# LiuShenLan/global_body_planner

Measured on AMD Instinct MI355X. Metric: valid extend-attempts/sec + time-to-first-solution, 1024×1024 rough_terrain, higher is better.
Workload: dtype f64; 1 GPU; config 3: synth-rough-1024, 262,144-attempt batch per GPU, isValidStateActionPair[Reverse] 50/50; terrain=synth-rough-1024, batch_per_gpu=262144, global_batch=262144, seed=20251018, kernel=persistent, waves=2, adaptive=False, terrain_storage=f32, parallelism=shard1 (no collective on the data path)

## Files before the change

### global_body_planner_amd/_lib.py

```python
import ctypes
import os

_HERE = os.path.dirname(os.path.abspath(__file__))
LIB_PATH = os.path.join(_HERE, "lib", "libgbp.so")

OK = 0
FLIGHT, STANCE, CONNECT_STANCE = 0, 1, 2
FORWARD, REVERSE = 0, 1
TRAPPED, ADVANCED, REACHED = 0, 1, 2
NUM_GEN_STATES = 6
F_VALID, F_OOD, F_NAN, F_SNEW_SET, F_TNEW_SET, F_FRAGILE, F_LIMIT, F_RESOLVED = 1, 2, 4, 8, 16, 32, 64, 128
MAX_SAMPLES = 7000
F_STAGE_SHIFT = 8
F_STAGE_MASK = 0xF << F_STAGE_SHIFT
STORAGE_AUTO, STORAGE_F32, STORAGE_F64 = 0, 1, 2
OPT_KERNEL, OPT_BLOCK, OPT_WAVES, OPT_LDS_COORDS, OPT_HELPERS = 1, 2, 4, 5, 8
OPT_AFFINE_COORDS, OPT_COORD_MODE, OPT_XCD_MAP, OPT_FAST_RCP, OPT_FRAGILE_EPS = 9, 10, 13, 14, 15
OPT_NN_STATS = 18
PLAN_HALT_TARGETS, PLAN_HALT_EXTEND, PLAN_HALT_CONNECT = 1, 2, 4
PLAN_HALT_STAR, PLAN_HALT_STAR_PAIRS = 8, 16
KERNEL_DIRECT, KERNEL_PERSISTENT = 0, 1

EXPORTS = [
    "gbp_version", "gbp_status_string", "gbp_device_count", "gbp_device_alloc",
    "gbp_device_free", "gbp_memcpy_h2d", "gbp_memcpy_d2h", "gbp_stream_synchronize",
    "gbp_terrain_create", "gbp_terrain_destroy", "gbp_terrain_info",
    "gbp_terrain_set_option", "gbp_terrain_get_option",
    "gbp_height_batch_dev", "gbp_height_batch_host",
    "gbp_normal_batch_dev", "gbp_normal_batch_host",
    "gbp_valid_states_dev", "gbp_valid_states_host",
    "gbp_validate_pairs_dev", "gbp_validate_pairs_host",
    "gbp_sample_states_dev", "gbp_sample_states_host", "gbp_sample_actions_dev",
    "gbp_sample_actions_host", "gbp_terrain_set_sampling", "gbp_terrain_get_sampling",
    "gbp_sample_states_dir_dev", "gbp_sample_states_dir_host", "gbp_sample_actions_dir_dev",
    "gbp_sample_actions_dir_host",
    "gbp_extend_batch_dev", "gbp_extend_batch_host",
    "gbp_nearest_batch_dev", "gbp_nearest_batch_host",
    "gbp_neighbors_batch_dev", "gbp_neighbors_batch_host", "gbp_knn_batch_dev", "gbp_knn_batch_host",
    "gbp_knn_yaw_batch_dev", "gbp_knn_yaw_batch_host", "gbp_host_yaw",
    "gbp_resolve_fragile_host", "gbp_resolve_fragile_states_host", "gbp_extend_resolve_host",
    "gbp_stream_create", "gbp_stream_destroy",
    "gbp_tree_create", "gbp_tree_destroy", "gbp_tree_init", "gbp_tree_reserve", "gbp_tree_capacity",
    "gbp_tree_size", "gbp_tree_read", "gbp_tree_append_host", "gbp_tree_load_host",
    "gbp_tree_device_ptrs", "gbp_vertex_map_order", "gbp_vertex_map_rank",
    "gbp_plan_ws_create", "gbp_plan_ws_destroy", "gbp_plan_reset", "gbp_plan_half_dev",
    "gbp_plan_halves_dev", "gbp_plan_star_config", "gbp_plan_stage_timing", "gbp_plan_stage_times",
    "gbp_plan_status_read", "gbp_plan_resolve_host", "gbp_extend_tree_dev",
    "gbp_extend_tree_finish_dev", "gbp_extend_tree_host", "gbp_tree_nearest_dev",
]


class Sampling(ctypes.Structure):
    _fields_ = [("state_flag", ctypes.c_int32), ("state_speed_direction", ctypes.c_int32),
                ("state_p", ctypes.c_double), ("action_flag", ctypes.c_int32),
                ("reserved", ctypes.c_int32), ("action_p", ctypes.c_double)]


def sampling(state_flag=False, state_p=0.05, speed_direction=False, action_flag=False,
             action_p=0.15):
    return Sampling(int(bool(state_flag)), int(bool(speed_direction)), float(state_p),
                    int(bool(action_flag)), 0, float(action_p))


class GbpError(RuntimeError):
    def __init__(self, status, what=""):
        self.status = status
        msg = _lib.gbp_status_string(status).decode() if _lib is not None else str(status)
        super().__init__(f"{what}: gbp status {status} ({msg})")


_lib = None


def load(path=None):
    global _lib
    if path is None and _lib is not None:
        return _lib
    p = path or LIB_PATH
    if not os.path.exists(p):
        raise FileNotFoundError(
            f"{p} is missing: build the HIP engine first "
            "(python -c 'import __graft_entry__ as g; g.build()')")
    L = ctypes.CDLL(p)
    P, I, I64, U64, SZ = ctypes.c_void_p, ctypes.c_int, ctypes.c_int64, ctypes.c_uint64, ctypes.c_size_t
    sig = {
        "gbp_version": (I, []),
        "gbp_status_string": (ctypes.c_char_p, [I]),
        "gbp_device_count": (I, [P]),
        "gbp_device_alloc": (I, [I, SZ, P]),
        "gbp_device_free": (I, [P]),
        "gbp_memcpy_h2d": (I, [P, P, SZ, P]),
        "gbp_memcpy_d2h": (I, [P, P, SZ, P]),
        "gbp_stream_synchronize": (I, [P]),
        "gbp_terrain_create": (I, [I, I, I, P, P, P, P, P, P, I, P]),
        "gbp_terrain_destroy": (I, [P]),
        "gbp_terrain_info": (I, [P, P, P, P, P, P]),
        "gbp_terrain_set_option": (I, [P, I, I64]),
        "gbp_terrain_get_option": (I, [P, I, P]),
        "gbp_height_batch_dev": (I, [P, I64, P, P, P, P, P]),
        "gbp_height_batch_host": (I, [P, I64, P, P, P, P]),
        "gbp_normal_batch_dev": (I, [P, I64, P, P, P, P]),
        "gbp_normal_batch_host": (I, [P, I64, P, P, P]),
        "gbp_valid_states_dev": (I, [P, I64, P, P, I, P, P, P, P]),
        "gbp_valid_states_host": (I, [P, I64, P, P, I, P, P, P]),
        "gbp_validate_pairs_dev": (I, [P, I64, P, P, P, I, I, P, P, P, P, P, P]),
        "gbp_validate_pairs_host": (I, [P, I64, P, P, P, I, I, P, P, P, P, P]),
        "gbp_sample_states_dev": (I, [P, I64, U64, U64, I64, I, I, P, P, P]),
        "gbp_sample_actions_dev": (I, [I64, P, U64, U64, I64, P, P]),
        "gbp_sample_states_host": (I, [P, I64, U64, U64, I64, I, I, P, P]),
        "gbp_sample_actions_host": (I, [P, I64, P, U64, U64, I64, P]),
        "gbp_terrain_set_sampling": (I, [P, P]),
        "gbp_terrain_get_sampling": (I, [P, P]),
        "gbp_sample_states_dir_dev": (I, [P, I64, U64, U64, I64, P, P, P, P, P]),
        "gbp_sample_states_dir_host": (I, [P, I64, U64, U64, I64, P, P, P, P]),
        "gbp_sample_actions_dir_dev": (I, [P, I64, P, P, P, P, I, P, U64, U64, I64, P, P]),
        "gbp_sample_actions_dir_host": (I, [P, I64, P, P, P, P, I, P, U64, U64, I64, P]),
        "gbp_extend_batch_dev": (I, [P, I64, P, P, P, I, I, U64, I64, P, P, P, P, P, P, P]),
        "gbp_extend_batch_host": (I, [P, I64, P, P, P, I, I, U64, I64, P, P, P, P, P, P]),
        "gbp_resolve_fragile_host": (I, [P, I64, P, P, P, I, I, P, P, P, P, P, P]),
        "gbp_resolve_fragile_states_host": (I, [P, I64, P, P, I, P, P, P, P]),
        "gbp_extend_resolve_host": (I, [P, I64, P, P, P, I, I, U64, I64, P, P, P, P, P, P, P]),
        "gbp_stream_create": (I, [I, P]),
        "gbp_stream_destroy": (I, [P]),
        "gbp_tree_create": (I, [I, I64, P]),
        "gbp_tree_destroy": (I, [P]),
        "gbp_tree_init": (I, [P, P, P]),
        "gbp_tree_reserve": (I, [P, I64, P]),
        "gbp_tree_capacity": (I, [P, P]),
        "gbp_tree_size": (I, [P, P, P]),
        "gbp_tree_read": (I, [P, I64, I64, P, P, P, P, P]),
        "gbp_tree_append_host": (I, [P, I64, P, P, P, P]),
        "gbp_tree_load_host": (I, [P, I64, P, P, P, P]),
        "gbp_vertex_map_order": (I, [I64, P]),
        "gbp_vertex_map_rank": (I, [I64, I64, P]),
        "gbp_tree_device_ptrs": (I, [P, P, P]),
        "gbp_plan_ws_create": (I, [P, I64, P]),
        "gbp_plan_ws_destroy": (I, [P]),
        "gbp_plan_reset": (I, [P, I64, P]),
        "gbp_plan_half_dev": (I, [P, P, P, P, ctypes.c_int32, I, I64, U64, U64, I64, I, I, P]),
        "gbp_plan_halves_dev": (I, [P, P, P, P, ctypes.c_int32, ctypes.c_int32, I64, U64, U64, U64,
                                    I, I, P]),
        "gbp_plan_status_read": (I, [P, P, P]),
        "gbp_plan_star_config": (I, [P, I, ctypes.c_double, I64, I64]),
        "gbp_plan_stage_timing": (I, [P, I]),
        "gbp_plan_stage_times": (I, [P, P, I, P, I]),
        "gbp_plan_resolve_host": (I, [P, P, P, P, I, I64, I, P, P, P]),
        "gbp_extend_tree_dev": (I, [P, P, P, I64, P, P, I, I, U64, I64, P, P, P]),
        "gbp_extend_tree_finish_dev": (I, [P, P, P, I64, I, P, P, P]),
        "gbp_extend_tree_host": (I, [P, P, P, I64, P, I, I, U64, I64, P, P, P]),
        "gbp_tree_nearest_dev": (I, [P, P, I64, P, P, P]),
        "gbp_nearest_batch_dev": (I, [I64, P, I64, P, P, P, P]),
# ... 28 lines not shown
```

### global_body_planner_amd/csrc/gbp_engine.hip

```cpp
#pragma clang fp contract(off)

#include <hip/hip_runtime.h>
#include <stdint.h>
#include <string.h>

#include <cstring>

#include <algorithm>
#include <cmath>
#include <mutex>
#include <new>
#include <vector>

#include "gbp.h"
#include "gbp_device.h"
#include "gbp_lane.h"
#include "gbp_um_order.h"
#include "gbp_internal.h"
#include "host/gbp_host_check.h"

using namespace gbp;

namespace {

// ... 62 lines not shown
    for (int k = 0; k < 8; k++) s[k] = states[8 * i + k];
    Acc acc{0, 0, 0};
    const bool v = is_valid_state(T, s, phase ? phase[i] : phase_all, acc);
    if (valid) valid[i] = v;
    if (flags) flags[i] = acc.flags | (v ? GBP_F_VALID : 0u);
    if (counts) counts[i] = (acc.G & 0xFFFFu) | (acc.V << 16);
  }
}

extern __shared__ double gbp_smem[];

template <class ZT, bool ADAPTIVE, int W, int CM>
__global__ __launch_bounds__(256, W) void k_validate_direct(
    TerrainView<ZT> T0, int64_t n, const double *__restrict__ S, const double *__restrict__ A,
    const uint8_t *__restrict__ dir, int dir_all, uint8_t *__restrict__ valid,
    double *__restrict__ s_new, double *__restrict__ t_new, uint32_t *__restrict__ flags,
    uint32_t *__restrict__ counts) {
  const TerrainView<ZT> T = CM == 1 ? stage_coords(T0, gbp_smem) : T0;
  const int64_t i = blockIdx.x * (int64_t)blockDim.x + threadIdx.x;
  if (i >= n) return;
  double s[8], a[10], sn[8];
#pragma unroll
  for (int k = 0; k < 8; k++) s[k] = S[8 * i + k];
#pragma unroll
  for (int k = 0; k < 10; k++) a[k] = A[10 * i + k];
  double tn = 0;
  Acc acc{0, 0, 0};
  uint32_t f = 0;
  const int d = dir ? dir[i] : dir_all;
  const bool v = (d == GBP_FORWARD) ? pair_forward<ZT, ADAPTIVE>(T, s, a, sn, tn, acc, f)
                                    : pair_reverse<ZT, ADAPTIVE>(T, s, a, sn, tn, acc, f);
  f |= acc.flags | (v ? GBP_F_VALID : 0u);
  if (valid) valid[i] = v;
  if (s_new && (f & GBP_F_SNEW_SET)) {
#pragma unroll
    for (int k = 0; k < 8; k++) s_new[8 * i + k] = sn[k];
  }
  if (t_new && (f & GBP_F_TNEW_SET)) t_new[i] = tn;
  flags[i] = f;
  if (counts) counts[i] = (acc.G & 0xFFFFu) | (acc.V << 16);
}



struct SnewRec {
  int idx, kind;
  double p;
};
constexpr int SN_RING = 2 * 64;

struct XBox {
  int seq, ack, fin, n_idle;
  unsigned long long act;
  int st[64];
  uint32_t vb[64], r0[64], r1[64];
  double t[64], ts[64];
};

#ifdef GBP_LOOP_PROF
__device__ unsigned long long gbp_loop_prof[8192 * 12];
#define LP_T(v) const unsigned long long v = __builtin_readcyclecounter()
#define LP_ADD(k, a, b) lp[k] += (b) - (a)
#else
#define LP_T(v)
#define LP_ADD(k, a, b)
#endif

template <class ZT, bool ADAPTIVE, int W, int CM, bool ONE>
__global__ __launch_bounds__(512, W) void k_validate_persistent(
    TerrainView<ZT> T0, int n, const double *__restrict__ S, const double *__restrict__ A,
    const uint8_t *__restrict__ dir, int dir_all, uint8_t *__restrict__ valid,
    double *__restrict__ s_new, double *__restrict__ t_new, uint32_t *__restrict__ flags,
    uint32_t *__restrict__ counts, const int *__restrict__ n_dev, int helpers, int xcd_map) {
#ifndef GBP_LDS_TERRAIN
  const TerrainView<ZT> T = CM == 1 ? stage_coords(T0, gbp_smem) : T0;
#else
  TerrainView<ZT> T = CM == 1 ? stage_coords(T0, gbp_smem) : T0;
  {
    ZT *zl = (ZT *)((SnewRec *)(gbp_smem + (CM == 1 ? (T0.nx + T0.ny + 1) & ~1 : 0) +
                                (size_t)blockDim.x * SA_ROW) +
                    (blockDim.x / WAVE) * SN_RING);
    const int nz = 2 * (T0.nx - 1) * T0.ny;
    typedef ZT zpair __attribute__((ext_vector_type(2)));
    for (int i = threadIdx.x; i < nz / 2; i += blockDim.x)
      ((zpair *)zl)[i] = ((const zpair *)T0.z)[i];
    __syncthreads();
#ifndef GBP_LDS_TERRAIN_STAGE_ONLY
    T.z = zl;
#endif
  }
#endif
  if (n_dev) n = *n_dev;
  const int lane = threadIdx.x & (WAVE - 1);
  const unsigned long long lt_mask = (1ull << lane) - 1ull;
  double *const SA = gbp_smem + (CM == 1 ? (T0.nx + T0.ny + 1) & ~1 : 0);
  double *const wave_rows = SA + (size_t)(threadIdx.x & ~(WAVE - 1)) * SA_ROW;
  SnewRec *const ring = (SnewRec *)(SA + (size_t)blockDim.x * SA_ROW) + (threadIdx.x / WAVE) * SN_RING;
  int ring_n = 0;
  auto flush = [&](int cnt) {
    if (lane < cnt) {
      const SnewRec r = ring[lane];
      double sv[8], av[10], o[8];
#pragma unroll
      for (int k = 0; k < 8; k++) sv[k] = S[8 * (size_t)r.idx + k];
#pragma unroll
      for (int k = 0; k < 10; k++) av[k] = A[10 * (size_t)r.idx + k];
      sample_state(sv, av,
                   r.kind == SN_STANCE_S ? ST_FWD_STANCE
                                         : (r.kind == SN_FLIGHT_B ? ST_FWD_LAND : ST_REV_STANCE),
                   r.p, o);
#pragma unroll
      for (int k = 0; k < 8; k++) s_new[8 * (size_t)r.idx + k] = o[k];
    }
  };
#ifdef GBP_XWAVE
  XBox *const xbox = (XBox *)((SnewRec *)(SA + (size_t)blockDim.x * SA_ROW) + (blockDim.x / WAVE) * SN_RING);
  const int wv = threadIdx.x / WAVE;
  XBox *const mybox = xbox + wv;
  XBox *const pbox = xbox + (wv ^ 1);
  const bool has_partner = (wv ^ 1) < (int)(blockDim.x / WAVE);
  double *const partner_rows = SA + (size_t)((wv ^ 1) * WAVE) * SA_ROW;
  if (lane == 0) {
    mybox->seq = 0;
    mybox->ack = 0;
    mybox->fin = 0;
  }
  __syncthreads();
  int myseq = 0, served = 0;
  bool fin_sent = false;
#endif
  Lane L;
  L.s = SA + (size_t)threadIdx.x * SA_ROW;
  L.a = L.s + 8;
  L.stage = ST_IDLE;
  unsigned int cur, end;
  {
    const unsigned int waves = gridDim.x * (blockDim.x / WAVE);
    const unsigned int wg = (xcd_map && (gridDim.x & 7u) == 0)
                                ? (blockIdx.x & 7u) * (gridDim.x >> 3) + (blockIdx.x >> 3)
                                : blockIdx.x;
    const unsigned int wid = wg * (blockDim.x / WAVE) + threadIdx.x / WAVE;
    cur = (unsigned int)(((unsigned long long)n * wid) / waves);
    end = (unsigned int)(((unsigned long long)n * (wid + 1)) / waves);
  }
#ifdef GBP_LOOP_PROF
  unsigned long long lp[12] = {0, 0, 0, 0, 0, 0, 0, 0, 0, 0, 0, 0};
  lp[8] = __builtin_amdgcn_s_memrealtime();
  LP_T(lp_start);
#endif
  for (;;) {
    LP_T(t0);
    const bool need = L.stage == ST_IDLE;
    unsigned long long m = __ballot(need);
    if (m && cur < end) {
      const unsigned int take = min(end - cur, (unsigned int)__popcll(m));
      const unsigned int rank = (unsigned int)__popcll(m & lt_mask);
      const bool mine = need && rank < take;
      if (mine) {
        const unsigned int i = cur + rank;
        L.idx = (int)i;
#pragma unroll
        for (int k = 0; k < 8; k++) L.s[k] = S[8 * (size_t)i + k];
#pragma unroll
        for (int k = 0; k < 10; k++) L.a[k] = A[10 * (size_t)i + k];
        L.f = 0;
        L.acc = Acc{0, 0, 0};
        L.snew_kind = SN_NONE;
        L.tnew_set = 0;
        const int d = dir ? dir[i] : dir_all;
        enter_stage(L, d == GBP_FORWARD ? ST_FWD_STANCE : ST_REV_FLIGHT);
      }
      cur += take;
    }
    const unsigned long long act = __ballot(L.stage != ST_IDLE);
#ifdef GBP_XWAVE
    bool serve = false;
    if (!act) {
      if (!has_partner) break;
      if (!fin_sent) {
        __builtin_amdgcn_fence(__ATOMIC_RELEASE, "workgroup");
        if (lane == 0) __hip_atomic_store(&mybox->fin, 1, __ATOMIC_RELEASE, __HIP_MEMORY_SCOPE_WORKGROUP);
        fin_sent = true;
      }
      int pseq, pfin;
      for (;;) {
        pseq = __builtin_amdgcn_readfirstlane(
            __hip_atomic_load(&pbox->seq, __ATOMIC_ACQUIRE, __HIP_MEMORY_SCOPE_WORKGROUP));
        pfin = __builtin_amdgcn_readfirstlane(
            __hip_atomic_load(&pbox->fin, __ATOMIC_ACQUIRE, __HIP_MEMORY_SCOPE_WORKGROUP));
        if (pseq != served || pfin) break;
        __builtin_amdgcn_s_sleep(1);
      }
      if (pseq == served) break;
      __builtin_amdgcn_fence(__ATOMIC_ACQUIRE, "workgroup");
      served = pseq;
      serve = true;
    }
#else
    if (!act) break;
#endif
    LP_T(t1);
    LP_ADD(0, t0, t1);
    const bool owner = L.stage != ST_IDLE;
    asm volatile("" ::: "memory");
    const int n_act = __popcll(act);
    const bool tail = helpers && n_act < WAVE;
    int st = L.stage, slot = 0;
    const double *ps = L.s;
    double t_eval = owner ? stage_time(L) : 0.0;
    uint32_t vbase = L.acc.V;
    bool has = owner;
#ifdef GBP_XWAVE
    bool xhelp = false;
    if (tail && !serve && has_partner) {
      xhelp = __builtin_amdgcn_readfirstlane(
                  __hip_atomic_load(&pbox->fin, __ATOMIC_ACQUIRE, __HIP_MEMORY_SCOPE_WORKGROUP)) != 0;
      if (xhelp) {
        mybox->st[lane] = L.stage;
        mybox->t[lane] = L.t;
        mybox->ts[lane] = L.ts;
        mybox->vb[lane] = L.acc.V;
        if (lane == 0) {
          mybox->act = act;
          mybox->n_idle = WAVE - n_act;
        }
        __builtin_amdgcn_fence(__ATOMIC_RELEASE, "workgroup");
        myseq++;
        if (lane == 0) __hip_atomic_store(&mybox->seq, myseq, __ATOMIC_RELEASE, __HIP_MEMORY_SCOPE_WORKGROUP);
      }
    }
    if (serve) {
      const unsigned long long pact = pbox->act;
      const int pn = __popcll(pact);
      const int j = pbox->n_idle + lane;
      const int src = nth_set_bit(pact, j % pn);
      slot = 1 + j / pn;
      ps = partner_rows + src * SA_ROW;
      st = pbox->st[src];
      double t = pbox->t[src], ts = pbox->ts[src];
      vbase = pbox->vb[src];
      has = true;
      for (int k = 0; k < slot && has; k++) has = advance_on_success<ADAPTIVE>(st, ps + 8, t, ts);
      t_eval = sample_time(st, ps + 8, t);
    } else
#endif
    if (tail) {
      const unsigned long long idle = ~act;
      const int j = __popcll(idle & lt_mask);
      const int src = owner ? lane : nth_set_bit(act, j % n_act);
      slot = owner ? 0 : 1 + j / n_act;
      ps = wave_rows + src * SA_ROW;
      st = __shfl(L.stage, src);
      double t = __shfl(L.t, src), ts = __shfl(L.ts, src);
      vbase = __shfl(L.acc.V, src);
      if (!owner) {
        has = true;
        for (int k = 0; k < slot && has; k++) has = advance_on_success<ADAPTIVE>(st, ps + 8, t, ts);
        t_eval = sample_time(st, ps + 8, t);
      }
    }
    LP_T(t2);
    LP_ADD(1, t1, t2);
    Acc acc_s{0, vbase + (uint32_t)slot, 0};
    bool ok = false;
    if (has) {
      double sc[8];
      sample_state(ps, ps + 8, st, t_eval, sc);
      ok = is_valid_state<ZT, CM, ONE>(T, sc, stage_phase(st), acc_s);
    }
    LP_T(t3);
    LP_ADD(2, t2, t3);
#ifdef GBP_XWAVE
    if (serve) {
      pbox->r0[lane] = (acc_s.flags & 0xFFFFu) | (ok ? 1u << 16 : 0u) | (has ? 1u << 17 : 0u) |
                       ((acc_s.V - (vbase + (uint32_t)slot)) << 18);
      pbox->r1[lane] = acc_s.G;
      __builtin_amdgcn_fence(__ATOMIC_RELEASE, "workgroup");
      if (lane == 0) __hip_atomic_store(&pbox->ack, served, __ATOMIC_RELEASE, __HIP_MEMORY_SCOPE_WORKGROUP);
      continue;
    }
#endif
    bool decided = false;
    if (owner) {
      L.acc.G += acc_s.G;
      L.acc.V = acc_s.V;
      L.acc.flags |= acc_s.flags;
      decided = (acc_s.flags & GBP_F_LIMIT) ? true : transition<ADAPTIVE>(L, ok);
    }
    if (tail) {
      const unsigned long long idle = ~act;
      const int n_idle = WAVE - n_act;
#ifdef GBP_XWAVE
      int n_help = n_idle;
      if (xhelp) {
        while (__builtin_amdgcn_readfirstlane(__hip_atomic_load(
                   &mybox->ack, __ATOMIC_ACQUIRE, __HIP_MEMORY_SCOPE_WORKGROUP)) != myseq)
          __builtin_amdgcn_s_sleep(1);
        __builtin_amdgcn_fence(__ATOMIC_ACQUIRE, "workgroup");
        n_help += WAVE;
      }
#else
      const int n_help = n_idle;
#endif
      const uint32_t w0 = (acc_s.flags & 0xFFFFu) | (ok ? 1u << 16 : 0u) | (has ? 1u << 17 : 0u) |
// ... 398 lines not shown
        ci = (int)j;
      }
      const double td = __shfl(kd, nk - 1);
      const int ti = __shfl(ki, nk - 1);
      if (!__ballot(knn_less(cd, ci, td, ti))) continue;
#pragma unroll
      for (int k = 2; k <= WAVE; k <<= 1)
#pragma unroll
        for (int jj = k >> 1; jj > 0; jj >>= 1) {
          const bool up = (lane & k) == 0;
          knn_cx(cd, ci, co, jj, ((lane & jj) == 0) == up);
        }
      {
        const double rd = __shfl(cd, WAVE - 1 - lane);
        const int ri = __shfl(ci, WAVE - 1 - lane);
        const double ro = __shfl(co, WAVE - 1 - lane);
        if (knn_less(rd, ri, kd, ki)) {
          kd = rd;
          ki = ri;
          od = ro;
        }
      }
#pragma unroll
      for (int jj = WAVE >> 1; jj > 0; jj >>= 1) knn_cx(kd, ki, od, jj, (lane & jj) == 0);
    }
    if (lane < nk) {
      const bool real = ki != 0x7FFFFFFF;
      out[qi * nk + lane] = real ? ki : -1;
      if (dist) dist[qi * nk + lane] = real ? od : __builtin_nan("");
    }
  }
}

}

namespace {

int coord_mode(const gbp_terrain *t, bool lds_ok) {
  if (lds_ok) return 1;
  return (t->opt_affine && t->affine) ? 2 : 0;
}

int validate_coord_mode(const gbp_terrain *t, bool direct) {
  const size_t rows =
      direct ? 0 : (sizeof(double) * SA_ROW + sizeof(SnewRec) * SN_RING / WAVE) * (size_t)t->opt_block;
  const size_t per_cu = std::max<int64_t>(1, t->opt_waves * 256 / t->opt_block) *
                        (stage_bytes(t->nx, t->ny) + rows);
  const bool lds_ok = t->opt_lds_coords && stage_bytes(t->nx, t->ny) + rows <= t->lds_max &&
                      (direct || per_cu <= 160 * 1024);
  if (!direct && !(t->one_x && t->one_y)) return 0;
  return coord_mode(t, lds_ok);
}

template <class ZT, bool AD, int W, int CM, bool ONE>
int launch_validate_w(gbp_terrain *t, int64_t n, const double *s, const double *a,
                      const uint8_t *dir, int dir_all, uint8_t *valid, double *s_new,
                      double *t_new, uint32_t *flags, uint32_t *counts, hipStream_t st,
                      const int *n_dev) {
  const TerrainView<ZT> T = view<ZT>(t);
  const int block = (int)t->opt_block;
  const size_t coords = CM == 1 ? stage_bytes(t->nx, t->ny) : 0;
  const size_t rows = sizeof(double) * SA_ROW * (size_t)block;
  const int64_t chunk = (int64_t)1 << 30;
  for (int64_t off = 0; off < n; off += chunk) {
    const int64_t m = std::min<int64_t>(n - off, chunk);
    const uint8_t *d = dir ? dir + off : nullptr;
    uint8_t *v = valid ? valid + off : nullptr;
    double *sn = s_new ? s_new + 8 * off : nullptr;
    double *tn = t_new ? t_new + off : nullptr;
    uint32_t *c = counts ? counts + off : nullptr;
    if (t->opt_kernel == GBP_KERNEL_DIRECT && !n_dev) {
      const int db = std::min(block, 256);
      const unsigned g = (unsigned)((m + db - 1) / db);
      hipLaunchKernelGGL((k_validate_direct<ZT, AD, 1, CM == 2 ? 0 : CM>), dim3(g), dim3(db), coords, st, T, m,
                         s + 8 * off, a + 10 * off, d, dir_all, v, sn, tn, flags + off, c);
    } else {
      const int64_t resident = (int64_t)t->num_cus * std::max<int64_t>(1, t->opt_waves * 256 / block);
      const int64_t g = std::max<int64_t>(1, std::min<int64_t>(resident, (m + WAVE - 1) / WAVE));
      const size_t ring = sizeof(SnewRec) * SN_RING * (size_t)(block / WAVE);
#ifdef GBP_LDS_TERRAIN
      const size_t zb = sizeof(ZT) * 2 * (size_t)(t->nx - 1) * t->ny;
      if (coords + rows + ring + zb > t->lds_max) return GBP_E_SHAPE;
#elif defined(GBP_XWAVE)
      const size_t zb = sizeof(XBox) * (size_t)(block / WAVE);
#else
      const size_t zb = 0;
#endif
      hipLaunchKernelGGL((k_validate_persistent<ZT, AD, W, CM, ONE>), dim3((unsigned)g), dim3(block),
                         coords + rows + ring + zb, st, T, (int)m, s + 8 * off, a + 10 * off, d, dir_all, v, sn, tn,
                         flags + off, c, n_dev, (int)t->opt_helpers,
                         (int)t->opt_xcd_map);
    }
    HIPCHK(hipGetLastError());
  }
  return GBP_OK;
}

template <class ZT>
int launch_validate(gbp_terrain *t, int64_t n, const double *s, const double *a,
                    const uint8_t *dir, int dir_all, int adaptive, uint8_t *valid,
                    double *s_new, double *t_new, uint32_t *flags, uint32_t *counts,
                    hipStream_t st, const int *n_dev = nullptr) {
#define GBP_LVW(AD, W, CM, ONE)                                                              \
  launch_validate_w<ZT, AD, W, CM, ONE>(t, n, s, a, dir, dir_all, valid, s_new, t_new, flags,  \
                                        counts, st, n_dev)
#define GBP_LV(AD, W)                                                                        \
  (cm == 2 ? GBP_LVW(AD, W, 2, true)                                                         \
   : cm == 1 ? GBP_LVW(AD, W, 1, true)                                                       \
             : (one ? GBP_LVW(AD, W, 0, true) : GBP_LVW(AD, W, 0, false)))
  const int64_t w = t->opt_waves;
  const int cm = validate_coord_mode(t, t->opt_kernel == GBP_KERNEL_DIRECT && !n_dev);
  const bool one = t->one_x && t->one_y;
  if (adaptive) return w >= 4 ? GBP_LV(true, 4) : (w == 3 ? GBP_LV(true, 3) : GBP_LV(true, 2));
  return w >= 4 ? GBP_LV(false, 4) : (w == 3 ? GBP_LV(false, 3) : GBP_LV(false, 2));
#undef GBP_LV
#undef GBP_LVW
}

bool valid_handle(const gbp_terrain *t) { return t != nullptr && t->d_z != nullptr; }

int guess_host(int n, double d0, double inv, double v) {
  const int i = (int)((v - d0) * inv);
  return i < 0 ? 0 : (i > n - 2 ? n - 2 : i);
}

int one_step_exact(const double *d, int n, double inv) {
  if (!(inv > 0) || !std::isfinite(inv)) return 0;
  for (int i = 0; i + 1 < n; i++) {
    if (!(d[i] < d[i + 1])) return 0;
    const int lo = guess_host(n, d[0], inv, d[i]);
    const int hi = guess_host(n, d[0], inv, std::nextafter(d[i + 1], -INFINITY));
    if (lo < i - 1 || hi > i + 1) return 0;
  }
  return 1;
}

bool affine_exact(const double *d, int n, double a, double h, int base) {
  for (int i = 0; i < n; i++) {
    const double v = a + h * (double)(i - base);
    if (memcmp(&v, &d[i], sizeof v) != 0) return false;
  }
  return true;
}

// ... 35 lines not shown
      for (int k = 0; k < 9; k++, hv = std::nextafter(hv, INFINITY)) {
        if (affine_exact(d, n, av, hv, bs)) {
          *a = av;
          *h = hv;
          *base = bs;
          return true;
        }
      }
    }
  }
  return false;
}

struct Stage {
  gbp_terrain *t;
  char *base;
  size_t off = 0;
  template <class T>
  T *take(size_t count) {
    off = (off + 255) & ~(size_t)255;
    T *p = (T *)(base + off);
    off += count * sizeof(T);
    return p;
  }
};
size_t rnd(size_t b) { return (b + 255) & ~(size_t)255; }

}

__attribute__((visibility("hidden"))) int gbp_internal_validate_dev_n(
    gbp_terrain *t, int64_t n_max, const int *n_dev, const double *s, const double *a,
    const uint8_t *dir, int dir_all, int adaptive, uint8_t *valid, double *s_new, double *t_new,
    uint32_t *flags, uint32_t *counts, hipStream_t st) {
  if (n_max <= 0) return GBP_OK;
  if (t->storage == GBP_STORAGE_F32)
    return launch_validate<float>(t, n_max, s, a, dir, dir_all, adaptive, valid, s_new, t_new,
                                  flags, counts, st, n_dev);
  return launch_validate<double>(t, n_max, s, a, dir, dir_all, adaptive, valid, s_new, t_new,
                                 flags, counts, st, n_dev);
}

extern "C" {

#ifdef GBP_LOOP_PROF
int gbp_loop_prof_read(unsigned long long *out, int n_waves) {
  if (!out || n_waves < 0 || n_waves > 8192) return GBP_E_INVALID_ARG;
  if (hipDeviceSynchronize() != hipSuccess) return GBP_E_HIP;
  if (hipMemcpyFromSymbol(out, HIP_SYMBOL(gbp_loop_prof), sizeof(unsigned long long) * 12 * n_waves) !=
      hipSuccess)
    return GBP_E_HIP;
  return GBP_OK;
}
#endif

int gbp_version(void) { return 200;  }

const char *gbp_status_string(int status) {
  switch (status) {
    case GBP_OK: return "ok";
    case GBP_E_INVALID_ARG: return "invalid argument";
    case GBP_E_BAD_HANDLE: return "bad handle";
    case GBP_E_ALLOC: return "device allocation failed";
    case GBP_E_HIP: return "HIP runtime error";
    case GBP_E_SHAPE: return "bad shape";
    case GBP_E_NO_DEVICE: return "no HIP device";
    case GBP_E_UNSUPPORTED: return "unsupported";
    default: return "unknown status";
  }
}

int gbp_device_count(int *count) {
  if (!count) return GBP_E_INVALID_ARG;
  int c = 0;
  if (hipGetDeviceCount(&c) != hipSuccess) c = 0;
  *count = c;
  return c > 0 ? GBP_OK : GBP_E_NO_DEVICE;
}

int gbp_device_alloc(int device, size_t bytes, void **ptr) {
  if (!ptr) return GBP_E_INVALID_ARG;
  DeviceGuard g(device);
  if (hipMalloc(ptr, bytes ? bytes : 1) != hipSuccess) return GBP_E_ALLOC;
  return GBP_OK;
}

int gbp_device_free(void *ptr) {
  if (ptr) HIPCHK(hipFree(ptr));
  return GBP_OK;
}

int gbp_memcpy_h2d(void *dst, const void *src, size_t bytes, gbp_stream stream) {
  HIPCHK(hipMemcpyAsync(dst, src, bytes, hipMemcpyHostToDevice, (hipStream_t)stream));
  return GBP_OK;
}

int gbp_memcpy_d2h(void *dst, const void *src, size_t bytes, gbp_stream stream) {
  HIPCHK(hipMemcpyAsync(dst, src, bytes, hipMemcpyDeviceToHost, (hipStream_t)stream));
  return GBP_OK;
}

int gbp_stream_synchronize(gbp_stream stream) {
  HIPCHK(hipStreamSynchronize((hipStream_t)stream));
  return GBP_OK;
}

int gbp_terrain_create(int device, int nx, int ny, const double *x, const double *y,
// ... 140 lines not shown
      return GBP_OK;
    case GBP_OPT_BLOCK:
      if (value < 64 || value > 512 || value % 64) return GBP_E_INVALID_ARG;
      t->opt_block = value;
      return GBP_OK;
    case GBP_OPT_WAVES:
      if (value < 1 || value > 4) return GBP_E_INVALID_ARG;
      t->opt_waves = value;
      return GBP_OK;
    case GBP_OPT_LDS_COORDS:
      t->opt_lds_coords = value ? 1 : 0;
      return GBP_OK;
    case GBP_OPT_HELPERS:
      t->opt_helpers = value ? 1 : 0;
      return GBP_OK;
    case GBP_OPT_AFFINE_COORDS:
      t->opt_affine = value ? 1 : 0;
      return GBP_OK;
    case GBP_OPT_XCD_MAP:
      t->opt_xcd_map = value ? 1 : 0;
      return GBP_OK;
    case GBP_OPT_FAST_RCP:
      t->opt_fast_rcp = value ? 1 : 0;
      return GBP_OK;
    case GBP_OPT_NN_STATS:
      t->opt_nn_stats = value ? 1 : 0;
      return GBP_OK;
    case GBP_OPT_FRAGILE_EPS:
      if (value < 1000 || value > 1000000000000000LL) return GBP_E_INVALID_ARG;
      t->fragile_eps = (double)value * 1e-15;
      return GBP_OK;
    default:
      return GBP_E_INVALID_ARG;
  }
}

int gbp_terrain_get_option(const gbp_terrain *t, int key, int64_t *value) {
  if (!valid_handle(t)) return GBP_E_BAD_HANDLE;
  if (!value) return GBP_E_INVALID_ARG;
  switch (key) {
    case GBP_OPT_KERNEL: *value = t->opt_kernel; return GBP_OK;
    case GBP_OPT_BLOCK: *value = t->opt_block; return GBP_OK;
    case GBP_OPT_WAVES: *value = t->opt_waves; return GBP_OK;
    case GBP_OPT_LDS_COORDS: *value = t->opt_lds_coords; return GBP_OK;
    case GBP_OPT_HELPERS: *value = t->opt_helpers; return GBP_OK;
    case GBP_OPT_AFFINE_COORDS: *value = t->opt_affine; return GBP_OK;
    case GBP_OPT_XCD_MAP: *value = t->opt_xcd_map; return GBP_OK;
    case GBP_OPT_FAST_RCP: *value = t->opt_fast_rcp ? (t->rcp_seed != 0.0 ? 1 : 0) : 0; return GBP_OK;
    case GBP_OPT_NN_STATS: *value = t->opt_nn_stats; return GBP_OK;
    case GBP_OPT_FRAGILE_EPS: *value = (int64_t)std::llround(t->fragile_eps * 1e15); return GBP_OK;
    case GBP_OPT_COORD_MODE:
      *value = validate_coord_mode(t, t->opt_kernel == GBP_KERNEL_DIRECT);
      return GBP_OK;
    default: return GBP_E_INVALID_ARG;
  }
}

int gbp_height_batch_dev(gbp_terrain *t, int64_t n, const double *xy, double *height,
                         uint8_t *is_nan, uint8_t *ood, gbp_stream stream) {
  if (!valid_handle(t)) return GBP_E_BAD_HANDLE;
  if (n < 0 || (n > 0 && !xy)) return GBP_E_INVALID_ARG;
  if (n == 0) return GBP_OK;
  DeviceGuard g(t->device);
  if (((uintptr_t)xy) % 16) return GBP_E_INVALID_ARG;
  const size_t cbytes = stage_bytes(t->nx, t->ny);
  const bool lds = t->opt_lds_coords && cbytes <= t->lds_max;
  const unsigned grid = grid_for(n, 256, t->num_cus * 8);
  const double2 *p = (const double2 *)xy;
  hipStream_t st = (hipStream_t)stream;
  const int cm = coord_mode(t, lds);
#define GBP_K1(ZT, CM)                                                                      \
  hipLaunchKernelGGL((k_height<ZT, CM>), dim3(grid), dim3(256), CM == 1 ? cbytes : 0, st, \
                     view<ZT>(t), n, p, height, is_nan, ood)
  if (t->storage == GBP_STORAGE_F32) {
    if (cm == 2) GBP_K1(float, 2);
    else if (cm == 1) GBP_K1(float, 1);
    else GBP_K1(float, 0);
  } else {
    if (cm == 2) GBP_K1(double, 2);
    else if (cm == 1) GBP_K1(double, 1);
    else GBP_K1(double, 0);
  }
#undef GBP_K1
  HIPCHK(hipGetLastError());
  return GBP_OK;
}

int gbp_normal_batch_dev(gbp_terrain *t, int64_t n, const double *xy, double *normal,
                         uint8_t *ood, gbp_stream stream) {
  if (!valid_handle(t)) return GBP_E_BAD_HANDLE;
  if (n < 0 || (n > 0 && (!xy || !normal))) return GBP_E_INVALID_ARG;
  if (n == 0) return GBP_OK;
  DeviceGuard g(t->device);
  const unsigned grid = grid_for(n, 256, t->num_cus * 16);
  if (t->storage == GBP_STORAGE_F32)
    hipLaunchKernelGGL(k_normal<float>, dim3(grid), dim3(256), 0, (hipStream_t)stream,
                       view<float>(t), n, xy, normal, ood);
  else
    hipLaunchKernelGGL(k_normal<double>, dim3(grid), dim3(256), 0, (hipStream_t)stream,
                       view<double>(t), n, xy, normal, ood);
  HIPCHK(hipGetLastError());
  return GBP_OK;
}

int gbp_valid_states_dev(gbp_terrain *t, int64_t n, const double *states, const uint8_t *phase,
                         int phase_all, uint8_t *valid, uint32_t *flags, uint32_t *counts,
// ... 738 lines not shown
```

### include/gbp.h

```cpp
#ifndef GBP_H
#define GBP_H

#include <stddef.h>
#include <stdint.h>

#ifdef __cplusplus
extern "C" {
#endif

#define GBP_OK              0
#define GBP_E_INVALID_ARG  (-1)
#define GBP_E_BAD_HANDLE   (-2)
#define GBP_E_ALLOC        (-3)
#define GBP_E_HIP          (-4)
#define GBP_E_SHAPE        (-5)
#define GBP_E_NO_DEVICE    (-6)
#define GBP_E_UNSUPPORTED  (-7)

#define GBP_FLIGHT          0
#define GBP_STANCE          1
#define GBP_CONNECT_STANCE  2
#define GBP_FORWARD         0
#define GBP_REVERSE         1
#define GBP_TRAPPED         0
// ... 11 lines not shown
#define GBP_F_SNEW_SET   (1u << 3)
#define GBP_F_TNEW_SET   (1u << 4)
#define GBP_F_FRAGILE    (1u << 5)
#define GBP_F_LIMIT      (1u << 6)
#define GBP_F_RESOLVED   (1u << 7)
#define GBP_MAX_SAMPLES  7000u
#define GBP_F_DEPTH_CAPPED (1u << 12)
#define GBP_F_STAGE_SHIFT 8u
#define GBP_F_STAGE_MASK  (0xFu << GBP_F_STAGE_SHIFT)
#define GBP_STAGE_FWD_STANCE 1u
#define GBP_STAGE_FWD_FLIGHT 2u
#define GBP_STAGE_FWD_LAND   3u
#define GBP_STAGE_REV_FLIGHT 4u
#define GBP_STAGE_REV_STANCE 5u
#define GBP_STAGE_REV_START  6u

#define GBP_COUNT_G(c) ((c) & 0xFFFFu)
#define GBP_COUNT_V(c) ((c) >> 16)

typedef struct gbp_terrain gbp_terrain;
typedef void *gbp_stream;

int         gbp_version(void);
const char *gbp_status_string(int status);
int         gbp_device_count(int *count);
int         gbp_device_alloc(int device, size_t bytes, void **ptr);
int         gbp_device_free(void *ptr);
int         gbp_memcpy_h2d(void *dst, const void *src, size_t bytes, gbp_stream stream);
int         gbp_memcpy_d2h(void *dst, const void *src, size_t bytes, gbp_stream stream);
int         gbp_stream_synchronize(gbp_stream stream);

#define GBP_STORAGE_AUTO 0
#define GBP_STORAGE_F32  1
#define GBP_STORAGE_F64  2

int gbp_terrain_create(int device, int nx, int ny, const double *x, const double *y,
                       const double *z, const double *dx, const double *dy,
                       const double *dz, int storage, gbp_terrain **out);
int gbp_terrain_destroy(gbp_terrain *t);
int gbp_terrain_info(const gbp_terrain *t, int *nx, int *ny, int *storage,
                     double bounds[4], int *device);

#define GBP_OPT_KERNEL        1
#define GBP_OPT_BLOCK         2
#define GBP_OPT_WAVES         4
#define GBP_OPT_LDS_COORDS    5
#define GBP_OPT_HELPERS       8
#define GBP_OPT_AFFINE_COORDS 9
#define GBP_OPT_COORD_MODE   10
#define GBP_OPT_XCD_MAP      13
#define GBP_OPT_FAST_RCP     14
#define GBP_OPT_FRAGILE_EPS  15
#define GBP_OPT_NN_STATS     18
#define GBP_KERNEL_DIRECT     0
#define GBP_KERNEL_PERSISTENT 1
int gbp_terrain_set_option(gbp_terrain *t, int key, int64_t value);
int gbp_terrain_get_option(const gbp_terrain *t, int key, int64_t *value);

int gbp_height_batch_dev(gbp_terrain *t, int64_t n, const double *xy, double *height,
                         uint8_t *is_nan, uint8_t *ood, gbp_stream stream);
int gbp_height_batch_host(gbp_terrain *t, int64_t n, const double *xy, double *height,
                          uint8_t *is_nan, uint8_t *ood);
int gbp_normal_batch_dev(gbp_terrain *t, int64_t n, const double *xy, double *normal,
                         uint8_t *ood, gbp_stream stream);
int gbp_normal_batch_host(gbp_terrain *t, int64_t n, const double *xy, double *normal,
                          uint8_t *ood);

int gbp_valid_states_dev(gbp_terrain *t, int64_t n, const double *states,
                         const uint8_t *phase, int phase_all, uint8_t *valid,
                         uint32_t *flags, uint32_t *counts, gbp_stream stream);
int gbp_valid_states_host(gbp_terrain *t, int64_t n, const double *states,
                          const uint8_t *phase, int phase_all, uint8_t *valid,
                          uint32_t *flags, uint32_t *counts);

int gbp_validate_pairs_dev(gbp_terrain *t, int64_t n, const double *s, const double *a,
                           const uint8_t *direction, int direction_all, int adaptive,
                           uint8_t *valid, double *s_new, double *t_new, uint32_t *flags,
                           uint32_t *counts, gbp_stream stream);
int gbp_validate_pairs_host(gbp_terrain *t, int64_t n, const double *s, const double *a,
                            const uint8_t *direction, int direction_all, int adaptive,
                            uint8_t *valid, double *s_new, double *t_new, uint32_t *flags,
                            uint32_t *counts);

int gbp_sample_states_dev(gbp_terrain *t, int64_t n, uint64_t seed, uint64_t stream_id,
                          int64_t index_base, int require_phase, int max_tries,
                          double *states, int32_t *tries, gbp_stream stream);
int gbp_sample_states_host(gbp_terrain *t, int64_t n, uint64_t seed, uint64_t stream_id,
                           int64_t index_base, int require_phase, int max_tries,
                           double *states, int32_t *tries);
int gbp_sample_actions_dev(int64_t n, const double *normals, uint64_t seed,
                           uint64_t stream_id, int64_t index_base, double *actions,
                           gbp_stream stream);
int gbp_sample_actions_host(gbp_terrain *t, int64_t n, const double *normals, uint64_t seed,
                            uint64_t stream_id, int64_t index_base, double *actions);

typedef struct {
  int32_t state_flag;
  int32_t state_speed_direction;
  double state_p;
  int32_t action_flag;
  int32_t reserved;
  double action_p;
} gbp_sampling;
int gbp_terrain_set_sampling(gbp_terrain *t, const gbp_sampling *cfg);
int gbp_terrain_get_sampling(const gbp_terrain *t, gbp_sampling *cfg);
int gbp_sample_states_dir_dev(gbp_terrain *t, int64_t n, uint64_t seed, uint64_t stream_id,
                              int64_t index_base, const gbp_sampling *cfg, const double *s_from,
                              const double *s_to, double *states, gbp_stream stream);
int gbp_sample_states_dir_host(gbp_terrain *t, int64_t n, uint64_t seed, uint64_t stream_id,
                               int64_t index_base, const gbp_sampling *cfg, const double *s_from,
// ... 157 lines not shown
```

Measured before the change: 2.854 billion extend-attempts/s.

## Prefetch upcoming state-action rows into LDS via async global_load_lds refill window

```diff
diff --git a/global_body_planner_amd/_lib.py b/global_body_planner_amd/_lib.py
--- a/global_body_planner_amd/_lib.py
+++ b/global_body_planner_amd/_lib.py
@@ -17,6 +17,7 @@
 OPT_KERNEL, OPT_BLOCK, OPT_WAVES, OPT_LDS_COORDS, OPT_HELPERS = 1, 2, 4, 5, 8
 OPT_AFFINE_COORDS, OPT_COORD_MODE, OPT_XCD_MAP, OPT_FAST_RCP, OPT_FRAGILE_EPS = 9, 10, 13, 14, 15
 OPT_NN_STATS = 18
+OPT_REFILL_WINDOW = 19
 PLAN_HALT_TARGETS, PLAN_HALT_EXTEND, PLAN_HALT_CONNECT = 1, 2, 4
 PLAN_HALT_STAR, PLAN_HALT_STAR_PAIRS = 8, 16
 KERNEL_DIRECT, KERNEL_PERSISTENT = 0, 1
@@ -25,7 +26,7 @@
     "gbp_version", "gbp_status_string", "gbp_device_count", "gbp_device_alloc",
     "gbp_device_free", "gbp_memcpy_h2d", "gbp_memcpy_d2h", "gbp_stream_synchronize",
     "gbp_terrain_create", "gbp_terrain_destroy", "gbp_terrain_info",
-    "gbp_terrain_set_option", "gbp_terrain_get_option",
+    "gbp_terrain_set_option", "gbp_terrain_get_option", "gbp_validate_lds_plan",
     "gbp_height_batch_dev", "gbp_height_batch_host",
     "gbp_normal_batch_dev", "gbp_normal_batch_host",
     "gbp_valid_states_dev", "gbp_valid_states_host",
@@ -97,6 +98,7 @@
         "gbp_terrain_info": (I, [P, P, P, P, P, P]),
         "gbp_terrain_set_option": (I, [P, I, I64]),
         "gbp_terrain_get_option": (I, [P, I, P]),
+        "gbp_validate_lds_plan": (I, [I, I, I64, I64, SZ, P, P, P]),
         "gbp_height_batch_dev": (I, [P, I64, P, P, P, P, P]),
         "gbp_height_batch_host": (I, [P, I64, P, P, P, P]),
         "gbp_normal_batch_dev": (I, [P, I64, P, P, P, P]),
diff --git a/global_body_planner_amd/csrc/gbp_engine.hip b/global_body_planner_amd/csrc/gbp_engine.hip
--- a/global_body_planner_amd/csrc/gbp_engine.hip
+++ b/global_body_planner_amd/csrc/gbp_engine.hip
@@ -138,7 +138,7 @@
 struct XBox {
   int seq, ack, fin, n_idle;
   unsigned long long act;
-  int st[64];
+  int st[64], row[64];
   uint32_t vb[64], r0[64], r1[64];
   double t[64], ts[64];
 };
@@ -152,20 +152,75 @@
 #define LP_ADD(k, a, b)
 #endif
 
+[[maybe_unused]] constexpr int PF_MAX = 32;
+
+inline size_t rows_bytes(int block, int pf) {
+  const size_t nwv = (size_t)(block / WAVE);
+  return sizeof(double) * SA_ROW * (size_t)(WAVE + pf) * nwv + sizeof(SnewRec) * SN_RING * nwv +
+         sizeof(int) * ((nwv * (size_t)pf + 1) & ~(size_t)1);
+}
+
+__device__ __forceinline__ void row_to_lds(const double *S, const double *A, const uint8_t *dir,
+                                           unsigned int i, double *row, int lane) {
+  const unsigned int lds = __builtin_amdgcn_readfirstlane(
+      (unsigned int)(uintptr_t)(__attribute__((address_space(3))) void *)row);
+  const uint32_t *src = lane < 16 ? (const uint32_t *)(S + 8 * (size_t)i) + lane
+                                  : (const uint32_t *)(A + 10 * (size_t)i) + (lane - 16);
+  unsigned int keep;
+  if (lane < 36)
+    asm volatile("s_mov_b32 %0, m0\n\ts_mov_b32 m0, %2\n\ts_nop 0\n\t"
+                 "global_load_lds_dword %1, off\n\ts_mov_b32 m0, %0"
+                 : "=&s"(keep) : "v"(src), "s"(lds) : "memory");
+  if (dir && lane == 36)
+    asm volatile("s_mov_b32 %0, m0\n\ts_mov_b32 m0, %2\n\ts_nop 0\n\t"
+                 "global_load_lds_ubyte %1, off\n\ts_mov_b32 m0, %0"
+                 : "=&s"(keep) : "v"(dir + i), "s"(lds) : "memory");
+}
+
 template <class ZT, bool ADAPTIVE, int W, int CM, bool ONE>
 __global__ __launch_bounds__(512, W) void k_validate_persistent(
     TerrainView<ZT> T0, int n, const double *__restrict__ S, const double *__restrict__ A,
     const uint8_t *__restrict__ dir, int dir_all, uint8_t *__restrict__ valid,
     double *__restrict__ s_new, double *__restrict__ t_new, uint32_t *__restrict__ flags,
-    uint32_t *__restrict__ counts, const int *__restrict__ n_dev, int helpers, int xcd_map) {
+    uint32_t *__restrict__ counts, const int *__restrict__ n_dev, int helpers, int xcd_map, int pf) {
+  if (n_dev) n = *n_dev;
+  const int lane = threadIdx.x & (WAVE - 1);
+  const unsigned long long lt_mask = (1ull << lane) - 1ull;
+  const int nwv = blockDim.x / WAVE, wv = __builtin_amdgcn_readfirstlane(threadIdx.x / WAVE);
+  double *const SA = gbp_smem + (CM == 1 ? (T0.nx + T0.ny + 1) & ~1 : 0);
+  double *const wave_rows = SA + (size_t)wv * (WAVE + pf) * SA_ROW;
+  SnewRec *const ring = (SnewRec *)(SA + (size_t)nwv * (WAVE + pf) * SA_ROW) + wv * SN_RING;
+  [[maybe_unused]] int *const Q = (int *)(ring + (nwv - wv) * SN_RING) + wv * pf;
+  [[maybe_unused]] void *const lds_extra = Q + (((nwv * pf + 1) & ~1) - wv * pf);
+  unsigned int cur, end;
+  {
+    const unsigned int waves = gridDim.x * (blockDim.x / WAVE);
+    const unsigned int wg = (xcd_map && (gridDim.x & 7u) == 0)
+                                ? (blockIdx.x & 7u) * (gridDim.x >> 3) + (blockIdx.x >> 3)
+                                : blockIdx.x;
+    const unsigned int wid = wg * (blockDim.x / WAVE) + wv;
+    cur = __builtin_amdgcn_readfirstlane((unsigned int)(((unsigned long long)n * wid) / waves));
+    end = __builtin_amdgcn_readfirstlane((unsigned int)(((unsigned long long)n * (wid + 1)) / waves));
+  }
+  auto load_row = [&](unsigned int i, double *r, int &d) {
+    if (dir) d = dir[i];
+#pragma unroll
+    for (int k = 0; k < 8; k++) r[k] = S[8 * (size_t)i + k];
+#pragma unroll
+    for (int k = 0; k < 10; k++) r[8 + k] = A[10 * (size_t)i + k];
+  };
+#ifdef GBP_REFILL_WINDOW
+  const unsigned int take0 = min(end - cur, (unsigned int)WAVE);
+  double row0[18];
+  int dir0 = dir_all;
+  if ((unsigned int)lane < take0) load_row(cur + lane, row0, dir0);
+#endif
 #ifndef GBP_LDS_TERRAIN
   const TerrainView<ZT> T = CM == 1 ? stage_coords(T0, gbp_smem) : T0;
 #else
   TerrainView<ZT> T = CM == 1 ? stage_coords(T0, gbp_smem) : T0;
   {
-    ZT *zl = (ZT *)((SnewRec *)(gbp_smem + (CM == 1 ? (T0.nx + T0.ny + 1) & ~1 : 0) +
-                                (size_t)blockDim.x * SA_ROW) +
-                    (blockDim.x / WAVE) * SN_RING);
+    ZT *zl = (ZT *)lds_extra;
     const int nz = 2 * (T0.nx - 1) * T0.ny;
     typedef ZT zpair __attribute__((ext_vector_type(2)));
     for (int i = threadIdx.x; i < nz / 2; i += blockDim.x)
@@ -176,12 +231,6 @@
 #endif
   }
 #endif
-  if (n_dev) n = *n_dev;
-  const int lane = threadIdx.x & (WAVE - 1);
-  const unsigned long long lt_mask = (1ull << lane) - 1ull;
-  double *const SA = gbp_smem + (CM == 1 ? (T0.nx + T0.ny + 1) & ~1 : 0);
-  double *const wave_rows = SA + (size_t)(threadIdx.x & ~(WAVE - 1)) * SA_ROW;
-  SnewRec *const ring = (SnewRec *)(SA + (size_t)blockDim.x * SA_ROW) + (threadIdx.x / WAVE) * SN_RING;
   int ring_n = 0;
   auto flush = [&](int cnt) {
     if (lane < cnt) {
@@ -200,12 +249,11 @@
     }
   };
 #ifdef GBP_XWAVE
-  XBox *const xbox = (XBox *)((SnewRec *)(SA + (size_t)blockDim.x * SA_ROW) + (blockDim.x / WAVE) * SN_RING);
-  const int wv = threadIdx.x / WAVE;
+  XBox *const xbox = (XBox *)lds_extra;
   XBox *const mybox = xbox + wv;
   XBox *const pbox = xbox + (wv ^ 1);
   const bool has_partner = (wv ^ 1) < (int)(blockDim.x / WAVE);
-  double *const partner_rows = SA + (size_t)((wv ^ 1) * WAVE) * SA_ROW;
+  double *const partner_rows = SA + (size_t)(wv ^ 1) * (WAVE + pf) * SA_ROW;
   if (lane == 0) {
     mybox->seq = 0;
     mybox->ack = 0;
@@ -216,19 +264,28 @@
   bool fin_sent = false;
 #endif
   Lane L;
-  L.s = SA + (size_t)threadIdx.x * SA_ROW;
+  int row = lane;
+  L.s = wave_rows + row * SA_ROW;
   L.a = L.s + 8;
   L.stage = ST_IDLE;
-  unsigned int cur, end;
-  {
-    const unsigned int waves = gridDim.x * (blockDim.x / WAVE);
-    const unsigned int wg = (xcd_map && (gridDim.x & 7u) == 0)
-                                ? (blockIdx.x & 7u) * (gridDim.x >> 3) + (blockIdx.x >> 3)
-                                : blockIdx.x;
-    const unsigned int wid = wg * (blockDim.x / WAVE) + threadIdx.x / WAVE;
-    cur = (unsigned int)(((unsigned long long)n * wid) / waves);
-    end = (unsigned int)(((unsigned long long)n * (wid + 1)) / waves);
-  }
+  auto start = [&](unsigned int i, int d) {
+    L.idx = (int)i;
+    L.f = 0;
+    L.acc = Acc{0, 0, 0};
+    L.snew_kind = SN_NONE;
+    L.tnew_set = 0;
+    enter_stage(L, d == GBP_FORWARD ? ST_FWD_STANCE : ST_REV_FLIGHT);
+  };
+#ifdef GBP_REFILL_WINDOW
+  unsigned int staged = 0, qh = 0;
+  if (lane < pf) Q[lane] = WAVE + lane;
+  if ((unsigned int)lane < take0) {
+#pragma unroll
+    for (int k = 0; k < 18; k++) L.s[k] = row0[k];
+    start(cur + lane, dir0);
+  }
+  cur += take0;
+#endif
 #ifdef GBP_LOOP_PROF
   unsigned long long lp[12] = {0, 0, 0, 0, 0, 0, 0, 0, 0, 0, 0, 0};
   lp[8] = __builtin_amdgcn_s_memrealtime();
@@ -242,22 +299,48 @@
       const unsigned int take = min(end - cur, (unsigned int)__popcll(m));
       const unsigned int rank = (unsigned int)__popcll(m & lt_mask);
       const bool mine = need && rank < take;
-      if (mine) {
-        const unsigned int i = cur + rank;
-        L.idx = (int)i;
-#pragma unroll
-        for (int k = 0; k < 8; k++) L.s[k] = S[8 * (size_t)i + k];
-#pragma unroll
-        for (int k = 0; k < 10; k++) L.a[k] = A[10 * (size_t)i + k];
-        L.f = 0;
-        L.acc = Acc{0, 0, 0};
-        L.snew_kind = SN_NONE;
-        L.tnew_set = 0;
-        const int d = dir ? dir[i] : dir_all;
-        enter_stage(L, d == GBP_FORWARD ? ST_FWD_STANCE : ST_REV_FLIGHT);
+      unsigned int ts = 0;
+#ifdef GBP_REFILL_WINDOW
+      ts = min(take, staged);
+      if (ts) {
+        asm volatile("s_waitcnt vmcnt(0)" ::: "memory");
+        if (mine && rank < ts) {
+          unsigned int p = qh + rank;
+          p -= p >= (unsigned int)pf ? (unsigned int)pf : 0u;
+          const int got = Q[p];
+          Q[p] = row;
+          row = got;
+          L.s = wave_rows + row * SA_ROW;
+          L.a = L.s + 8;
+          start(cur + rank, dir ? ((const int *)L.s)[36] & 0xFF : dir_all);
+        }
+        qh += ts;
+        qh -= qh >= (unsigned int)pf ? (unsigned int)pf : 0u;
+        staged -= ts;
+      }
+#endif
+      if (mine && rank >= ts) {
+        double r[18];
+        int d = dir_all;
+        load_row(cur + rank, r, d);
+#pragma unroll
+        for (int k = 0; k < 18; k++) L.s[k] = r[k];
+        start(cur + rank, d);
       }
       cur += take;
     }
+#ifdef GBP_REFILL_WINDOW
+    if (pf && min(end - cur, (unsigned int)pf) > staged) {
+      const unsigned int want = min(end - cur, (unsigned int)pf);
+      const int qv = Q[lane < pf ? lane : 0];
+      for (unsigned int k = staged; k < want; k++) {
+        unsigned int p = qh + k;
+        p -= p >= (unsigned int)pf ? (unsigned int)pf : 0u;
+        row_to_lds(S, A, dir, cur + k, wave_rows + __builtin_amdgcn_readlane(qv, p) * SA_ROW, lane);
+      }
+      staged = want;
+    }
+#endif
     const unsigned long long act = __ballot(L.stage != ST_IDLE);
 #ifdef GBP_XWAVE
     bool serve = false;
@@ -303,6 +386,7 @@
                   __hip_atomic_load(&pbox->fin, __ATOMIC_ACQUIRE, __HIP_MEMORY_SCOPE_WORKGROUP)) != 0;
       if (xhelp) {
         mybox->st[lane] = L.stage;
+        mybox->row[lane] = row;
         mybox->t[lane] = L.t;
         mybox->ts[lane] = L.ts;
         mybox->vb[lane] = L.acc.V;
@@ -321,7 +405,7 @@
       const int j = pbox->n_idle + lane;
       const int src = nth_set_bit(pact, j % pn);
       slot = 1 + j / pn;
-      ps = partner_rows + src * SA_ROW;
+      ps = partner_rows + pbox->row[src] * SA_ROW;
       st = pbox->st[src];
       double t = pbox->t[src], ts = pbox->ts[src];
       vbase = pbox->vb[src];
@@ -335,7 +419,7 @@
       const int j = __popcll(idle & lt_mask);
       const int src = owner ? lane : nth_set_bit(act, j % n_act);
       slot = owner ? 0 : 1 + j / n_act;
-      ps = wave_rows + src * SA_ROW;
+      ps = wave_rows + __shfl(row, src) * SA_ROW;
       st = __shfl(L.stage, src);
       double t = __shfl(L.t, src), ts = __shfl(L.ts, src);
       vbase = __shfl(L.acc.V, src);
@@ -840,6 +924,27 @@
   return coord_mode(t, lds_ok);
 }
 
+inline size_t variant_lds(const gbp_terrain *t) {
+#ifdef GBP_XWAVE
+  return sizeof(XBox) * (size_t)(t->opt_block / WAVE);
+#else
+  return 0;
+#endif
+}
+
+int refill_window(const gbp_terrain *t, size_t coords, size_t extra) {
+#if !defined(GBP_REFILL_WINDOW) || defined(GBP_LDS_TERRAIN)
+  return 0;
+#else
+  const int block = (int)t->opt_block;
+  const size_t wgs = (size_t)std::max<int64_t>(1, t->opt_waves * 256 / block);
+  const size_t cap = std::min<size_t>(t->lds_max, 160 * 1024 / wgs);
+  for (int pf = PF_MAX; pf > 0; pf--)
+    if (coords + rows_bytes(block, pf) + extra <= cap) return pf;
+  return 0;
+#endif
+}
+
 template <class ZT, bool AD, int W, int CM, bool ONE>
 int launch_validate_w(gbp_terrain *t, int64_t n, const double *s, const double *a,
                       const uint8_t *dir, int dir_all, uint8_t *valid, double *s_new,
@@ -848,7 +953,6 @@
   const TerrainView<ZT> T = view<ZT>(t);
   const int block = (int)t->opt_block;
   const size_t coords = CM == 1 ? stage_bytes(t->nx, t->ny) : 0;
-  const size_t rows = sizeof(double) * SA_ROW * (size_t)block;
   const int64_t chunk = (int64_t)1 << 30;
   for (int64_t off = 0; off < n; off += chunk) {
     const int64_t m = std::min<int64_t>(n - off, chunk);
@@ -865,19 +969,16 @@
     } else {
       const int64_t resident = (int64_t)t->num_cus * std::max<int64_t>(1, t->opt_waves * 256 / block);
       const int64_t g = std::max<int64_t>(1, std::min<int64_t>(resident, (m + WAVE - 1) / WAVE));
-      const size_t ring = sizeof(SnewRec) * SN_RING * (size_t)(block / WAVE);
 #ifdef GBP_LDS_TERRAIN
       const size_t zb = sizeof(ZT) * 2 * (size_t)(t->nx - 1) * t->ny;
-      if (coords + rows + ring + zb > t->lds_max) return GBP_E_SHAPE;
-#elif defined(GBP_XWAVE)
-      const size_t zb = sizeof(XBox) * (size_t)(block / WAVE);
+      if (coords + rows_bytes(block, 0) + zb > t->lds_max) return GBP_E_SHAPE;
 #else
-      const size_t zb = 0;
+      const size_t zb = variant_lds(t);
 #endif
+      const int pf = refill_window(t, coords, zb);
       hipLaunchKernelGGL((k_validate_persistent<ZT, AD, W, CM, ONE>), dim3((unsigned)g), dim3(block),
-                         coords + rows + ring + zb, st, T, (int)m, s + 8 * off, a + 10 * off, d, dir_all, v, sn, tn,
-                         flags + off, c, n_dev, (int)t->opt_helpers,
-                         (int)t->opt_xcd_map);
+                         coords + rows_bytes(block, pf) + zb, st, T, (int)m, s + 8 * off, a + 10 * off, d, dir_all,
+                         v, sn, tn, flags + off, c, n_dev, (int)t->opt_helpers, (int)t->opt_xcd_map, pf);
     }
     HIPCHK(hipGetLastError());
   }
@@ -1019,6 +1120,27 @@
   return GBP_OK;
 }
 #endif
+
+int gbp_validate_lds_plan(int nx, int ny, int64_t block, int64_t waves, size_t lds_max,
+                          int *coord_lds, int *window, size_t *bytes) {
+  if (nx < 2 || ny < 2 || block < WAVE || block > 512 || block % WAVE || waves < 1)
+    return GBP_E_INVALID_ARG;
+  gbp_terrain t;
+  t.nx = nx;
+  t.ny = ny;
+  t.one_x = t.one_y = 1;
+  t.opt_affine = 0;
+  t.opt_block = block;
+  t.opt_waves = waves;
+  t.lds_max = lds_max;
+  const int cm = validate_coord_mode(&t, false);
+  const size_t coords = cm == 1 ? stage_bytes(nx, ny) : 0;
+  const int pf = refill_window(&t, coords, variant_lds(&t));
+  if (coord_lds) *coord_lds = cm == 1;
+  if (window) *window = pf;
+  if (bytes) *bytes = coords + rows_bytes((int)block, pf) + variant_lds(&t);
+  return GBP_OK;
+}
 
 int gbp_version(void) { return 200;  }
 
@@ -1265,6 +1387,10 @@
     case GBP_OPT_COORD_MODE:
       *value = validate_coord_mode(t, t->opt_kernel == GBP_KERNEL_DIRECT);
       return GBP_OK;
+    case GBP_OPT_REFILL_WINDOW:
+      *value = refill_window(t, validate_coord_mode(t, false) == 1 ? stage_bytes(t->nx, t->ny) : 0,
+                             variant_lds(t));
+      return GBP_OK;
     default: return GBP_E_INVALID_ARG;
   }
 }
diff --git a/include/gbp.h b/include/gbp.h
--- a/include/gbp.h
+++ b/include/gbp.h
@@ -87,10 +87,13 @@
 #define GBP_OPT_FAST_RCP     14
 #define GBP_OPT_FRAGILE_EPS  15
 #define GBP_OPT_NN_STATS     18
+#define GBP_OPT_REFILL_WINDOW 19
 #define GBP_KERNEL_DIRECT     0
 #define GBP_KERNEL_PERSISTENT 1
 int gbp_terrain_set_option(gbp_terrain *t, int key, int64_t value);
 int gbp_terrain_get_option(const gbp_terrain *t, int key, int64_t *value);
+int gbp_validate_lds_plan(int nx, int ny, int64_t block, int64_t waves, size_t lds_max,
+                          int *coord_lds, int *window, size_t *bytes);
 
 int gbp_height_batch_dev(gbp_terrain *t, int64_t n, const double *xy, double *height,
                          uint8_t *is_nan, uint8_t *ood, gbp_stream stream);
```

New measurement: 2.917 billion extend-attempts/s (median of 6 runs). 2.2% higher.
